# JuliaHealth/Thunderbolt.jl

Hardware: AMD Instinct MI355X
Metric: element-integrations/sec + DoF-updates/sec, 10M-hex Q1 monodomain (higher is better)
Workload: dtype f64

## Files before the change

### thunderbolt.jl_amd/csrc/tb_assembly.hip

```cpp
#include <hip/hip_runtime.h>

#include <cmath>
#include <cstring>
#include <type_traits>

#include "tb_elem.hpp"
#include "tb_forms.hpp"
#include "tb_hex8_sumfac.hpp"
#include "tb_internal.h"
#include "tb_math.hpp"

namespace tb {
using namespace tbk;

template <int NB> __host__ __device__ constexpr int sym_idx(int i, int j)
{
    return i <= j ? i * NB - (i * (i - 1)) / 2 + (j - i) : j * NB - (j * (j - 1)) / 2 + (i - j);
}

template <class E>
__device__ __forceinline__ void load_coords(const MeshView &m, int64_t cell, double (&x)[E::NV][3])
{
    int32_t nodes[E::NV];
    const int32_t *c = m.conn + cell * E::NV;
// ... 66 lines not shown
#pragma unroll
            for (int m = 0; m < 3; ++m)
#pragma unroll
                for (int l = 0; l < 3; ++l) H[m][l] = g.Jinv[m][0] * D[0][l] + g.Jinv[m][1] * D[1][l] + g.Jinv[m][2] * D[2][l];
#pragma unroll
            for (int m = 0; m < 3; ++m)
#pragma unroll
                for (int n = (SYM ? m : 0); n < 3; ++n)
                    G[m][n] = mw * (H[m][0] * g.Jinv[n][0] + H[m][1] * g.Jinv[n][1] + H[m][2] * g.Jinv[n][2]);
            if constexpr (SYM) { G[1][0] = G[0][1]; G[2][0] = G[0][2]; G[2][1] = G[1][2]; }
#pragma unroll
            for (int i = 0; i < NB; ++i) {
                double T[3];
#pragma unroll
                for (int m = 0; m < 3; ++m) T[m] = G[m][0] * tb.dN[q][i][0] + G[m][1] * tb.dN[q][i][1] + G[m][2] * tb.dN[q][i][2];
#pragma unroll
                for (int j = SYM ? i : 0; j < NB; ++j) {
                    double &k = Ke[SYM ? sym_idx<NB>(i, j) : i * NB + j];
                    k += tb.dN[q][j][0] * T[0];
                    k += tb.dN[q][j][1] * T[1];
                    k += tb.dN[q][j][2] * T[2];
                }
            }
        }
    }
    return ok;
}

template <class E>
__global__ void __launch_bounds__(256)
k_tabulate_spectral(const double *__restrict__ field, int64_t n_cells, double l0, double l1, double l2, double scale, double *__restrict__ dtab)
{
    const int64_t cell = (int64_t)blockIdx.x * blockDim.x + threadIdx.x;
    if (cell >= n_cells) return;
    constexpr int NB = E::NB;
    const Tables<E> &tb = g_tables<E>;
    double fc[NB * 9];
#pragma unroll
    for (int k = 0; k < NB * 9; ++k) fc[k] = field[cell * (NB * 9) + k];
#pragma unroll 1
    for (int q = 0; q < E::NQ; ++q) {
        double f[3] = {0, 0, 0}, s[3] = {0, 0, 0}, n[3] = {0, 0, 0};
#pragma unroll
        for (int a = 0; a < NB; ++a) {
            const double Na = tb.N[q][a];
#pragma unroll
            for (int d = 0; d < 3; ++d) {
                f[d] += Na * fc[9 * a + d];
                s[d] += Na * fc[9 * a + 3 + d];
                n[d] += Na * fc[9 * a + 6 + d];
            }
        }
        orthonormal_frame(f, s, n);
        double *o = dtab + (cell * E::NQ + q) * 6;
        int k = 0;
#pragma unroll
        for (int i = 0; i < 3; ++i)
#pragma unroll
            for (int j = i; j < 3; ++j) o[k++] = (l0 * f[i] * f[j] + l1 * s[i] * s[j] + l2 * n[i] * n[j]) * scale;
    }
}

template <class E>
__global__ void __launch_bounds__(256)
k_tabulate_isotropic(const double *__restrict__ field, int64_t n_cells, double scale, double *__restrict__ dtab)
{
    const int64_t cell = (int64_t)blockIdx.x * blockDim.x + threadIdx.x;
    if (cell >= n_cells) return;
    constexpr int NB = E::NB;
    const Tables<E> &tb = g_tables<E>;
    double fc[NB];
#pragma unroll
    for (int k = 0; k < NB; ++k) fc[k] = field[cell * NB + k];
    for (int q = 0; q < E::NQ; ++q) {
        double v = 0.0;
#pragma unroll
        for (int a = 0; a < NB; ++a) v += tb.N[q][a] * fc[a];
        v *= scale;
        double *o = dtab + (cell * E::NQ + q) * 6;
        o[0] = v; o[1] = 0.0; o[2] = 0.0; o[3] = v; o[4] = 0.0; o[5] = v;
    }
}

__device__ __forceinline__ double eval_source(const FormArgs &fa, const double (&xq)[3], int64_t cell, int q, int nq)
{
    switch (fa.src_kind) {
    case TB_SRC_CONST: return fa.p0;
    case TB_SRC_NORM_PLUS_T: return sqrt(xq[0] * xq[0] + xq[1] * xq[1] + xq[2] * xq[2]) + (fa.tslot ? fa.tslot[0] : fa.t);
    case TB_SRC_COS_EXP:
        return (fa.tslot ? fa.tslot[1] : fa.ct) * exp_b(-(xq[0] * xq[0] + xq[1] * xq[1] + xq[2] * xq[2]));
    case TB_SRC_TABULATED: return fa.table[cell * nq + q];
    }
    return 0.0;
}

template <class E>
__device__ __forceinline__ bool element_source(const double (&x)[E::NV][3], const FormArgs &fa, int64_t cell, double (&be)[E::NB])
{
    const Tables<E> &tb = g_tables<E>;
    GeoCoeffs<E> gc;
    geo_prepare(x, gc);
    bool ok = true;
#pragma unroll 1
    for (int q = 0; q < E::NQ; ++q) {
        Geom g;
        geometry_rt<E>(tb, q, gc, g);
        ok = ok && (g.dOmega > 0.0);
        double xq[3];
        geo_position(gc, tb, q, xq);
        const double fw = eval_source(fa, xq, cell, q, E::NQ) * g.dOmega;
#pragma unroll
        for (int j = 0; j < E::NB; ++j) be[j] += fw * tb.N[q][j];
    }
    return ok;
}

__device__ __forceinline__ void flag_neg_detj(Status *st, int64_t cell)
{
    st->neg_detj = 1;
    st->cell = cell;
}

template <class MapT>
__global__ void k_build_emap(const int32_t *__restrict__ cell_dofs, int64_t n_cells, int ndpc,
                             const int64_t *__restrict__ rowptr, const int32_t *__restrict__ colidx, MapT *__restrict__ emap,
                             Status *st)
{
    const int64_t tid = (int64_t)blockIdx.x * blockDim.x + threadIdx.x;
    if (tid >= n_cells * ndpc) return;
    const int64_t cell = tid % n_cells;
    const int i = (int)(tid / n_cells);
    const int32_t *d = cell_dofs + cell * ndpc;
    const int32_t row = d[i];
    const int64_t lo0 = rowptr[row], hi0 = rowptr[row + 1];
    for (int j = 0; j < ndpc; ++j) {
        const int32_t c = d[j];
        int64_t lo = lo0, hi = hi0;
        while (lo < hi) {
            const int64_t mid = (lo + hi) >> 1;
            if (colidx[mid] < c) lo = mid + 1; else hi = mid;
        }
        if (lo >= hi0 || colidx[lo] != c) { st->pattern_missing = 1; st->cell = cell; lo = lo0; }
        emap[(int64_t)(i * ndpc + j) * n_cells + cell] = (MapT)lo;
    }
}

template <class E, int FORM, bool FIELD, bool SYM, class MapT>
__global__ void __launch_bounds__(128)
k_matrix_direct(MeshView m, FormArgs fa, const MapT *__restrict__ emap, const int32_t *__restrict__ list, int64_t n,
                double *__restrict__ nz, int atomic, Status *st)
{
    constexpr int NB = E::NB;
    const int64_t tid = (int64_t)blockIdx.x * blockDim.x + threadIdx.x;
    if (tid >= n) return;
    const int64_t cell = list ? list[tid] : tid;
    double x[E::NV][3];
    load_coords<E>(m, cell, x);
    double Ke[SYM ? NB * (NB + 1) / 2 : NB * NB];
#pragma unroll
    for (int k = 0; k < (SYM ? NB * (NB + 1) / 2 : NB * NB); ++k) Ke[k] = 0.0;
    if (!element_matrix<E, FORM, FIELD, SYM>(x, fa, cell, Ke)) flag_neg_detj(st, cell);
    const MapT *mp = emap + cell;
#pragma unroll
    for (int i = 0; i < NB; ++i)
#pragma unroll
        for (int j = 0; j < NB; ++j) {
            const double v = Ke[SYM ? sym_idx<NB>(i, j) : i * NB + j];
            const int64_t k = (int64_t)mp[(int64_t)(i * NB + j) * m.n_cells];
            if (atomic) unsafeAtomicAdd(nz + k, v); else nz[k] += v;
        }
}

template <class E>
__global__ void __launch_bounds__(256)
// ... 94 lines not shown
        if (!element_matrix<E, FORM, FIELD, SYM>(x, fa, cell, Ke)) flag_neg_detj(st, cell);
#ifdef TB_ABLATION
        if (!(fa.debug & 1))
#endif
#pragma unroll
        for (int i = 0; i < NB; ++i) {
            if (ro[i] == 0xFFFF) continue;
            double *row = acc + ro[i];
#pragma unroll
            for (int j = 0; j < NB; ++j) unsafeAtomicAdd(row + cp[i * NB + j], Ke[SYM ? sym_idx<NB>(i, j) : i * NB + j]);
        }
        if (!more) break;
        e = en; cell = celln;
#pragma unroll
        for (int a_ = 0; a_ < E::NV; ++a_) { x[a_][0] = xn[a_][0]; x[a_][1] = xn[a_][1]; x[a_][2] = xn[a_][2]; }
    }
    __syncthreads();

#ifdef TB_ABLATION
    if (fa.debug & 1) { if (threadIdx.x == 0) nz[p] = acc[0] + Ke_sink(); }
    if (fa.debug & 2) return;
#endif
    const int half = threadIdx.x >> 5, hl = threadIdx.x & 31, nhalves = T >> 5;
#pragma unroll 4
    for (int s = half; s < nrows; s += nhalves) {
        const int64_t g0 = dnz[s];
        const uint2 ol = dol[s];
        double *dst = nz + g0;
        for (uint32_t k = hl; k < ol.y; k += 32) dst[k] = acc[ol.x + k];
    }
}

template <class E>
__global__ void __launch_bounds__(PATCH_MAX_THREADS)
k_vector_patch(MeshView m, FormArgs fa, PatchView pv, double *__restrict__ b, Status *st)
{
    extern __shared__ double acc[];
    const int T = blockDim.x;
    const int64_t p = blockIdx.x;
    const int64_t e0 = pv.elem_ptr[p], e1 = pv.elem_ptr[p + 1];
    const int64_t r0 = pv.row_ptr[p], r1 = pv.row_ptr[p + 1];
    const int nrows = (int)(r1 - r0);
    int64_t e = e0 + threadIdx.x;
    int64_t cell = 0;
    double x[E::NV][3];
    if (e < e1) { cell = pv.elem_cell[e]; load_coords<E>(m, cell, x); }
    for (int k = threadIdx.x; k < nrows; k += T) acc[k] = 0.0;
    __syncthreads();
    while (e < e1) {
        const int64_t en = e + T;
        const bool more = en < e1;
        int64_t celln = 0;
        double xn[E::NV][3];
        if (more) { celln = pv.elem_cell[en]; load_coords<E>(m, celln, xn); }
        uint16_t lr[E::NB];
        const uint16_t *lp = pv.elem_lrow + e * E::NB;
#pragma unroll
        for (int j = 0; j < E::NB; ++j) lr[j] = lp[j];
        double be[E::NB];
#pragma unroll
        for (int j = 0; j < E::NB; ++j) be[j] = 0.0;
        if (!element_source<E>(x, fa, cell, be)) flag_neg_detj(st, cell);
#pragma unroll
        for (int j = 0; j < E::NB; ++j)
            if (lr[j] != 0xFFFF) unsafeAtomicAdd(&acc[lr[j]], be[j]);
        if (!more) break;
        e = en; cell = celln;
#pragma unroll
        for (int a_ = 0; a_ < E::NV; ++a_) { x[a_][0] = xn[a_][0]; x[a_][1] = xn[a_][1]; x[a_][2] = xn[a_][2]; }
    }
    __syncthreads();
    for (int s = threadIdx.x; s < nrows; s += T) b[pv.row_dof[r0 + s]] = acc[s];
}

struct VecPatchView {
    const uint4 *hdr;
    const uint16_t *elem_ln;
    const int32_t *elem_cell;
    const double *pcoord;
    const int32_t *pdof;
    int max_nodes;
};

template <bool HALO>
__global__ void __launch_bounds__(256, 3)
k_vector_hex8_patch(FormArgs fa, VecPatchView pv, double *__restrict__ b, Status *st)
{
    extern __shared__ double lds[];
    constexpr int T = 256, NI = 2, NX = 13, ND = 3;
    const int tid = threadIdx.x;
    const uint4 h = pv.hdr[blockIdx.x];
    const int64_t e0 = h.x, n0 = h.y;
    const int nrows = (int)(h.z & 0xffff), nnodes = (int)(h.z >> 16), ne = (int)h.w;
    double *acc = lds;
    double *xs = lds + pv.max_nodes;
    uint4 lnv[NI];
#pragma unroll
    for (int k = 0; k < NI; ++k) lnv[k] = tid + k * T < ne ? ((const uint4 *)pv.elem_ln)[e0 + tid + k * T] : make_uint4(0, 0, 0, 0);
    const double *pc = pv.pcoord + 3 * n0;
    double xc[NX];
#pragma unroll
    for (int j = 0; j < NX; ++j) xc[j] = tid + j * T < 3 * nnodes ? pc[tid + j * T] : 0.0;
    const int32_t *pd = pv.pdof + n0;
    int32_t dofs[ND];
#pragma unroll
    for (int j = 0; j < ND; ++j) dofs[j] = tid + j * T < nrows ? pd[tid + j * T] : 0;
    for (int k = tid; k < nnodes; k += T) acc[k] = 0.0;
#pragma unroll
    for (int j = 0; j < NX; ++j) if (tid + j * T < 3 * nnodes) xs[tid + j * T] = xc[j];
    for (int k = tid + NX * T; k < 3 * nnodes; k += T) xs[k] = pc[k];
    __syncthreads();
#pragma unroll 1
    for (int it = 0, ei = tid; ei < ne; ++it, ei += T) {
        const uint4 l4 = it < NI ? lnv[0] : ((const uint4 *)pv.elem_ln)[e0 + ei];
#pragma unroll
        for (int k = 0; k + 1 < NI; ++k) lnv[k] = lnv[k + 1];
        const uint32_t ln[8] = {l4.x & 0xffffu, l4.x >> 16, l4.y & 0xffffu, l4.y >> 16, l4.z & 0xffffu, l4.z >> 16, l4.w & 0xffffu, l4.w >> 16};
        double x[8][3];
#pragma unroll
        for (int a = 0; a < 8; ++a) {
            const double *px = xs + 3 * ln[a];
            x[a][0] = px[0]; x[a][1] = px[1]; x[a][2] = px[2];
        }
        int64_t cell = 0;
        if (fa.src_kind == TB_SRC_TABULATED) cell = pv.elem_cell[e0 + ei];
        double be[8];
        if (!hex8_sf_source(x, [&](int q, const double(&xq)[3]) { return eval_source(fa, xq, cell, q, 8); }, be)) flag_neg_detj(st, pv.elem_cell[e0 + ei]);
#pragma unroll
        for (int a = 0; a < 8; ++a)
            if (!HALO || ln[a] < (uint32_t)nrows) unsafeAtomicAdd(acc + ln[a], be[a]);
    }
    __syncthreads();
#pragma unroll
    for (int j = 0; j < ND; ++j)
        if (tid + j * T < nrows) {
            if (HALO) b[dofs[j]] = acc[tid + j * T];
            else unsafeAtomicAdd(b + dofs[j], acc[tid + j * T]);
        }
    for (int k = tid + ND * T; k < nrows; k += T) {
        if (HALO) b[pd[k]] = acc[k];
        else unsafeAtomicAdd(b + pd[k], acc[k]);
    }
}


static inline unsigned nblocks(int64_t n, int bs) { return (unsigned)((n + bs - 1) / bs); }

int ensure_emap(tb_pattern *p)
{
    if (p->d_emap) return TB_OK;
    tb_mesh *m = p->mesh;
    tb_device *dev = m->dev;
    const int64_t n = m->n_cells * m->ndpc;
    p->map64 = p->nnz >= (int64_t)0x7fffffff;
    const size_t bytes = (size_t)m->n_cells * m->ndpc * m->ndpc * (p->map64 ? 8 : 4);
    TB_HIP(hipMalloc(&p->d_emap, bytes));
    int rc = reset_status(dev);
    if (rc) return rc;
    if (p->map64)
        hipLaunchKernelGGL(k_build_emap<int64_t>, dim3(nblocks(n, 256)), dim3(256), 0, dev->stream, m->d_cell_dofs, m->n_cells,
                           m->ndpc, p->d_rowptr, p->d_colidx, (int64_t *)p->d_emap, dev->d_status);
    else
        hipLaunchKernelGGL(k_build_emap<int32_t>, dim3(nblocks(n, 256)), dim3(256), 0, dev->stream, m->d_cell_dofs, m->n_cells,
                           m->ndpc, p->d_rowptr, p->d_colidx, (int32_t *)p->d_emap, dev->d_status);
    TB_HIP(hipGetLastError());
    return check_status(dev);
}

static PatchView make_patch_view(const tb_mesh *m, const tb_pattern *p)
{
    const PatchPlan *pp = m->patches.get();
    PatchView v{};
    v.elem_ptr = pp->d_elem_ptr; v.row_ptr = pp->d_row_ptr; v.elem_cell = pp->d_elem_cell;
    v.elem_lrow = pp->d_elem_lrow; v.row_dof = pp->d_row_dof;
    if (p) {
        const PatchMatPlan *pm = p->patch_mat.get();
        v.row_desc = pm->d_row_desc;
        v.elem_rowoff = pm->d_elem_rowoff;
        v.colpos = pm->d_colpos8 ? (const void *)pm->d_colpos8 : (const void *)pm->d_colpos16;
        v.lds_entries = pm->max_lds_entries;
        v.max_rows = pp->max_rows;
    }
    return v;
}

template <class E, int FORM, bool FIELD, bool SYM>
static int run_matrix(tb_form *f, tb_pattern *p, int strategy, double t, double *d_nz)
{
    tb_mesh *m = f->mesh;
    tb_device *dev = m->dev;
    const MeshView mv = make_view(m);
    const FormArgs fa = make_args(f, t);
    if (strategy == TB_STRATEGY_PATCH) {
        { int rc = ensure_patch_plans(m, p); if (rc) return rc; }
        const PatchView pv = make_patch_view(m, p);
        const size_t lds = (size_t)p->patch_mat->max_lds_entries * sizeof(double) + (size_t)m->patches->max_rows * 16;
        const int T = m->patches->threads;
        auto launch = [&](auto k) -> int {
            TB_HIP(hipFuncSetAttribute((const void *)k, hipFuncAttributeMaxDynamicSharedMemorySize, (int)lds));
            hipLaunchKernelGGL(k, dim3((unsigned)m->patches->n_patches), dim3(T), lds, dev->stream, mv, fa, pv, d_nz, dev->d_status);
            return TB_OK;
        };
        int rc;
        if (p->patch_mat->d_colpos8) rc = launch(k_matrix_patch<E, FORM, FIELD, SYM, uint8_t, 2>);
        else rc = launch(k_matrix_patch<E, FORM, FIELD, SYM, uint16_t, 2>);
        if (rc) return rc;
        TB_HIP(hipGetLastError());
        return TB_OK;
    }
    { int rc = ensure_emap(p); if (rc) return rc; }
    TB_HIP(hipMemsetAsync(d_nz, 0, (size_t)p->nnz * sizeof(double), dev->stream));
    auto go = [&](const int32_t *list, int64_t n, int atomic) -> int {
        if (n == 0) return TB_OK;
        if (p->map64)
            hipLaunchKernelGGL((k_matrix_direct<E, FORM, FIELD, SYM, int64_t>), dim3(nblocks(n, 128)), dim3(128), 0, dev->stream, mv, fa,
                               (const int64_t *)p->d_emap, list, n, d_nz, atomic, dev->d_status);
        else
            hipLaunchKernelGGL((k_matrix_direct<E, FORM, FIELD, SYM, int32_t>), dim3(nblocks(n, 128)), dim3(128), 0, dev->stream, mv, fa,
                               (const int32_t *)p->d_emap, list, n, d_nz, atomic, dev->d_status);
        TB_HIP(hipGetLastError());
        return TB_OK;
    };
// ... 792 lines not shown
    }
    __syncthreads();
    const int quarter = tid >> 4, ql = tid & 15;
    for (int s = quarter; s < nrows; s += T / 16) {
        const uint4 d = desc[s];
        const int64_t g0 = (int64_t)(((uint64_t)d.y << 32) | d.x);
        for (uint32_t k = ql; k < d.w; k += 16) {
            if constexpr (WK) nzK[g0 + k] = accK[d.z + k];
            if constexpr (WM) nzM[g0 + k] = accM[d.z + k];
        }
    }
}

bool tet4_patch_applicable(const tb_form *f, const tb_pattern *)
{
    static const bool legacy = getenv("TB_PATCH_KERNEL") && !strcmp(getenv("TB_PATCH_KERNEL"), "legacy");
    if (legacy) return false;
    const tb_mesh *m = f->mesh;
    if (m->field_kind != TB_TET4 || m->geom_kind != TB_TET4 || m->ncomp != 1 || f->qorder != 2 || f->has_cellset) return false;
    if (f->kind == TB_FORM_DIFFUSION) return !f->field;
    return f->kind == TB_FORM_MASS;
}

int launch_assemble_tet4_patch(tb_form *fK, tb_form *fM, tb_pattern *p, double t, double *d_nzK, double *d_nzM)
{
    tb_form *any = fK ? fK : fM;
    tb_mesh *m = any->mesh;
    tb_device *dev = m->dev;
    int rc = reset_status(dev);
    if (rc) return rc;
    const int nreg = fK && fM ? 2 : 1;
    rc = ensure_patch_fused(m, p, nreg);
    if (rc) return rc;
    const PatchPlan *pp = m->patches.get();
    const PatchFusedPlan *pf = p->patch_fused.get();
    if (!pf->d_hdr) { set_error("tetrahedron patch kernel: a patch exceeds the packed header (1023 rows / 2047 nodes / 2047 instances)"); return TB_ERR_UNSUPPORTED; }
    TetPatchView pv{pf->d_elem_ln, pf->d_elem_sig, pf->d_sigtab, pf->d_row_desc, pp->d_elem_cell, pf->max_lds_entries, pp->max_rows, pf->max_nodes};
    const size_t lds = (size_t)nreg * pv.kcap * sizeof(double) + (size_t)pv.max_rows * sizeof(RowDesc) + (size_t)pv.max_nodes * 3 * sizeof(double);
    const FormArgs aK = fK ? make_args(fK, t) : FormArgs{}, aM = fM ? make_args(fM, t) : FormArgs{};
    const bool fm = fM && fM->field;
    auto launch = [&](auto k) -> int {
        TB_HIP(hipFuncSetAttribute((const void *)k, hipFuncAttributeMaxDynamicSharedMemorySize, (int)lds));
        hipLaunchKernelGGL(k, dim3((unsigned)pp->n_patches), dim3(256), lds, dev->stream, aK, aM, pv, (const uint4 *)pf->d_hdr, pf->d_pcoord, d_nzK, d_nzM, dev->d_status);
        return TB_OK;
    };
    if (fK && fM) rc = fm ? launch(k_patch_tet4<true, true, true>) : launch(k_patch_tet4<true, true, false>);
    else if (fK) rc = launch(k_patch_tet4<true, false, false>);
    else rc = fm ? launch(k_patch_tet4<false, true, true>) : launch(k_patch_tet4<false, true, false>);
    if (rc) return rc;
    TB_HIP(hipGetLastError());
    return check_status(dev);
}

int launch_assemble_matrix(tb_form *f, tb_pattern *p, int strategy, double t, double *d_nz)
{
    tb_mesh *m = f->mesh;
    int rc = reset_status(m->dev);
    if (rc) return rc;
    if (strategy == TB_STRATEGY_ELEMENT && m->field_kind != TB_HEX27) strategy = TB_STRATEGY_PER_COLOR;
    if (strategy == TB_STRATEGY_PATCH && hex8_patch_applicable(f, p)) {
        rc = f->kind == TB_FORM_DIFFUSION ? launch_assemble_hex8_patch(f, nullptr, p, t, d_nz, nullptr) : launch_assemble_hex8_patch(nullptr, f, p, t, nullptr, d_nz);
        if (rc != TB_ERR_UNSUPPORTED) return rc;
        rc = reset_status(m->dev);
        if (rc) return rc;
    }
    if (strategy == TB_STRATEGY_PATCH && tet4_patch_applicable(f, p)) {
        rc = f->kind == TB_FORM_DIFFUSION ? launch_assemble_tet4_patch(f, nullptr, p, t, d_nz, nullptr) : launch_assemble_tet4_patch(nullptr, f, p, t, nullptr, d_nz);
        if (rc != TB_ERR_UNSUPPORTED) return rc;
        rc = reset_status(m->dev);
        if (rc) return rc;
    }
    if (m->field_kind == TB_HEX8 && f->qorder == 2) rc = run_matrix_form<Hex8<2>>(f, p, strategy, t, d_nz);
    else if (m->field_kind == TB_TET4 && f->qorder == 2) rc = run_matrix_form<Tet4<2>>(f, p, strategy, t, d_nz);
    else if (m->field_kind == TB_QUAD4 && f->qorder == 2) rc = run_matrix_form<Quad4<2>>(f, p, strategy, t, d_nz);
    else if (m->field_kind == TB_HEX27 && f->qorder == 3) rc = run_q2(f, p, strategy, t, d_nz, nullptr);
    else {
        set_error("matrix assembly: field kind %d with quadrature order %d not implemented", m->field_kind, f->qorder);
        return TB_ERR_UNSUPPORTED;
    }
    if (rc) return rc;
    return check_status(m->dev);
}

template <class E>
static int run_vector(tb_form *f, int strategy, double t, double *d_b)
{
    tb_mesh *m = f->mesh;
    tb_device *dev = m->dev;
    const MeshView mv = make_view(m);
    const FormArgs fa = make_args(f, t);
    static const bool legacy_vec = tune_env("TB_VECTOR_KERNEL") && !strcmp(tune_env("TB_VECTOR_KERNEL"), "legacy");
    if constexpr (std::is_same<E, Hex8<2>>::value) {
        if (!legacy_vec && !f->has_cellset && (strategy == TB_STRATEGY_PATCH || strategy == TB_STRATEGY_ATOMIC)) {
            const bool halo = strategy == TB_STRATEGY_PATCH;
            int rc = ensure_vec_patch_plan(m, halo);
            if (rc == TB_OK) {
                const VecPatchPlan *vp = m->vpatches[halo].get();
                const VecPatchView pv{(const uint4 *)vp->d_hdr, vp->d_elem_ln, vp->d_elem_cell, vp->d_pcoord, vp->d_pdof, vp->max_nodes};
                const size_t lds = (size_t)vp->max_nodes * 4 * sizeof(double);
                if (!halo) TB_HIP(hipMemsetAsync(d_b, 0, (size_t)m->ndofs * sizeof(double), dev->stream));
                if (halo) {
                    TB_HIP(hipFuncSetAttribute((const void *)k_vector_hex8_patch<true>, hipFuncAttributeMaxDynamicSharedMemorySize, (int)lds));
                    hipLaunchKernelGGL(k_vector_hex8_patch<true>, dim3((unsigned)vp->n_patches), dim3(256), lds, dev->stream, fa, pv, d_b, dev->d_status);
                } else {
                    TB_HIP(hipFuncSetAttribute((const void *)k_vector_hex8_patch<false>, hipFuncAttributeMaxDynamicSharedMemorySize, (int)lds));
                    hipLaunchKernelGGL(k_vector_hex8_patch<false>, dim3((unsigned)vp->n_patches), dim3(256), lds, dev->stream, fa, pv, d_b, dev->d_status);
                }
                TB_HIP(hipGetLastError());
                return TB_OK;
            }
            if (rc != TB_ERR_UNSUPPORTED) return rc;
        }
    }
    if (strategy == TB_STRATEGY_PATCH) {
        { int rc = ensure_patch_plans(m, nullptr); if (rc) return rc; }
        const PatchView pv = make_patch_view(m, nullptr);
        const int T = m->patches->threads;
        hipLaunchKernelGGL((k_vector_patch<E>), dim3((unsigned)m->patches->n_patches), dim3(T),
                           (size_t)m->patches->max_rows * sizeof(double), dev->stream, mv, fa, pv, d_b, dev->d_status);
        TB_HIP(hipGetLastError());
        return TB_OK;
    }
    if (strategy == TB_STRATEGY_ELEMENT) {
        if (!m->ea) { int rc = build_ea_plan(m); if (rc) return rc; }
        hipLaunchKernelGGL((k_vector_direct<E>), dim3(nblocks(m->n_cells, 256)), dim3(256), 0, dev->stream, mv, fa,
                           (const int32_t *)nullptr, m->n_cells, d_b, m->ea->d_ea, 2, dev->d_status);
        TB_HIP(hipGetLastError());
        hipLaunchKernelGGL(k_ea_gather, dim3(nblocks(m->ndofs, 256)), dim3(256), 0, dev->stream, m->ea->d_ptr, m->ea->d_src,
                           m->ea->d_ea, m->ndofs, d_b);
        TB_HIP(hipGetLastError());
        return TB_OK;
    }
    TB_HIP(hipMemsetAsync(d_b, 0, (size_t)m->ndofs * sizeof(double), dev->stream));
    if (strategy == TB_STRATEGY_ATOMIC) {
        hipLaunchKernelGGL((k_vector_direct<E>), dim3(nblocks(m->n_cells, 256)), dim3(256), 0, dev->stream, mv, fa,
                           (const int32_t *)nullptr, m->n_cells, d_b, (double *)nullptr, 0, dev->d_status);
        TB_HIP(hipGetLastError());
        return TB_OK;
    }
    if (strategy == TB_STRATEGY_PER_COLOR) {
        if (!m->colors) { int rc = build_color_plan(m); if (rc) return rc; }
        for (int c = 0; c < m->colors->ncolors; ++c) {
            const int64_t n = m->colors->offsets[c + 1] - m->colors->offsets[c];
            if (!n) continue;
            hipLaunchKernelGGL((k_vector_direct<E>), dim3(nblocks(n, 256)), dim3(256), 0, dev->stream, mv, fa,
                               (const int32_t *)(m->colors->d_cells + m->colors->offsets[c]), n, d_b, (double *)nullptr, 1, dev->d_status);
            TB_HIP(hipGetLastError());
        }
        return TB_OK;
    }
    set_error("vector assembly: unknown strategy %d", strategy);
    return TB_ERR_UNSUPPORTED;
}

int launch_assemble_vector(tb_form *f, int strategy, double t, double *d_b)
{
    tb_mesh *m = f->mesh;
    int rc = reset_status(m->dev);
    if (rc) return rc;
    if (m->ncomp != 1) { set_error("source assembly needs a scalar field"); return TB_ERR_UNSUPPORTED; }
    if (m->field_kind == TB_HEX8 && f->qorder == 2) rc = run_vector<Hex8<2>>(f, strategy, t, d_b);
    else if (m->field_kind == TB_HEX8 && f->qorder == 3) rc = run_vector<Hex8<3>>(f, strategy, t, d_b);
    else if (m->field_kind == TB_TET4 && f->qorder == 2) rc = run_vector<Tet4<2>>(f, strategy, t, d_b);
    else if (m->field_kind == TB_QUAD4 && f->qorder == 2) rc = run_vector<Quad4<2>>(f, strategy, t, d_b);
    else if (m->field_kind == TB_HEX27 && f->qorder == 3) rc = run_q2(f, nullptr, strategy, t, nullptr, d_b);
    else {
        set_error("vector assembly: field kind %d with quadrature order %d not implemented", m->field_kind, f->qorder);
        return TB_ERR_UNSUPPORTED;
    }
    if (rc) return rc;
    return check_status(m->dev);
}

}
```

### thunderbolt.jl_amd/csrc/tb_hex8_sumfac.hpp

```cpp
#pragma once
#include "tb_elem.hpp"

namespace tbk {

struct SF {
    static constexpr double g = 0.5773502691896258;
    static constexpr double p = 0.5 * (1.0 + g), m = 0.5 * (1.0 - g);
    TB_HD static constexpr int bit(int a, int d) { return Hex8<2>::sgn(a, d) > 0 ? 1 : 0; }
    TB_HD static constexpr double f(int b, int qb) { return b == qb ? p : m; }
    TB_HD static constexpr double w(int t, int qb) { return t == 1 ? p * m : (t == 0 ? f(0, qb) * f(0, qb) : f(1, qb) * f(1, qb)); }
    TB_HD static constexpr int ty(int i, int j, int d) { return bit(i, d) + bit(j, d); }
    TB_HD static constexpr int sg(int i, int j, int d, int e) { return Hex8<2>::sgn(i, d) * Hex8<2>::sgn(j, e); }
};

__device__ __forceinline__ double sf_rcp(double y)
{
    double r = __builtin_amdgcn_rcp(y);
    r = fma(fma(-y, r, 1.0), r, r);
    r = fma(fma(-y, r, 1.0), r, r);
    return r;
}

template <bool WANT_K, bool FENCE, bool DIAG = false, bool ISO = false, class DFn>
__device__ __forceinline__ bool hex8_sf_geometry(const double (&x)[8][3], DFn &&Dq, double (&G)[8][6], double (&dq)[8], double sfac = -0.25)
// ... 42 lines not shown
            const double s = sfac * sf_rcp(det);
            double H[3][3];
#pragma unroll
            for (int a = 0; a < 3; ++a) {
                if constexpr (DIAG) {
                    H[a][0] = A[a][0] * D[0]; H[a][1] = A[a][1] * D[3]; H[a][2] = A[a][2] * D[5];
                } else {
                    H[a][0] = A[a][0] * D[0] + A[a][1] * D[1] + A[a][2] * D[2];
                    H[a][1] = A[a][0] * D[1] + A[a][1] * D[3] + A[a][2] * D[4];
                    H[a][2] = A[a][0] * D[2] + A[a][1] * D[4] + A[a][2] * D[5];
                }
            }
            int k = 0;
#pragma unroll
            for (int a = 0; a < 3; ++a)
#pragma unroll
                for (int b = a; b < 3; ++b) G[q][k++] = s * (H[a][0] * A[b][0] + H[a][1] * A[b][1] + H[a][2] * A[b][2]);
        }
        if constexpr (FENCE) __builtin_amdgcn_sched_barrier(0);
    }
    return ok;
}

template <int COMP, int DIR>
__device__ __forceinline__ void hex8_sf_diag(const double (&G)[8][6], double (&Y)[3][3])
{
    constexpr int E = DIR == 0 ? 1 : 0, F = DIR == 2 ? 1 : 2;
    double S[2][2];
#pragma unroll
    for (int qf = 0; qf < 2; ++qf)
#pragma unroll
        for (int qe = 0; qe < 2; ++qe) S[qf][qe] = G[(qe << E) | (qf << F)][COMP] + G[(qe << E) | (qf << F) | (1 << DIR)][COMP];
    double T[3][2];
#pragma unroll
    for (int qf = 0; qf < 2; ++qf) {
        T[0][qf] = fma(SF::w(0, 1), S[qf][1], SF::w(0, 0) * S[qf][0]);
        T[1][qf] = SF::w(1, 0) * (S[qf][0] + S[qf][1]);
        T[2][qf] = fma(SF::w(2, 1), S[qf][1], SF::w(2, 0) * S[qf][0]);
    }
#pragma unroll
    for (int te = 0; te < 3; ++te) {
        Y[te][0] = fma(SF::w(0, 1), T[te][1], SF::w(0, 0) * T[te][0]);
        Y[te][1] = SF::w(1, 0) * (T[te][0] + T[te][1]);
        Y[te][2] = fma(SF::w(2, 1), T[te][1], SF::w(2, 0) * T[te][0]);
    }
}
template <int COMP, int D, int E>
__device__ __forceinline__ void hex8_sf_cross(const double (&G)[8][6], double (&X)[2][2][3])
{
    constexpr int F = 3 - D - E;
    double A1[2][2][2];
#pragma unroll
    for (int qe = 0; qe < 2; ++qe)
#pragma unroll
        for (int qf = 0; qf < 2; ++qf) {
            const double g0 = G[(qe << E) | (qf << F)][COMP], g1 = G[(qe << E) | (qf << F) | (1 << D)][COMP];
            A1[0][qe][qf] = fma(SF::f(0, 1), g1, SF::f(0, 0) * g0);
            A1[1][qe][qf] = fma(SF::f(1, 1), g1, SF::f(1, 0) * g0);
        }
    double B1[2][2][2];
#pragma unroll
    for (int a = 0; a < 2; ++a)
#pragma unroll
        for (int qf = 0; qf < 2; ++qf) {
            B1[a][0][qf] = fma(SF::f(0, 1), A1[a][1][qf], SF::f(0, 0) * A1[a][0][qf]);
            B1[a][1][qf] = fma(SF::f(1, 1), A1[a][1][qf], SF::f(1, 0) * A1[a][0][qf]);
        }
#pragma unroll
    for (int a = 0; a < 2; ++a)
#pragma unroll
        for (int b = 0; b < 2; ++b) {
            X[a][b][0] = fma(SF::w(0, 1), B1[a][b][1], SF::w(0, 0) * B1[a][b][0]);
            X[a][b][1] = SF::w(1, 0) * (B1[a][b][0] + B1[a][b][1]);
            X[a][b][2] = fma(SF::w(2, 1), B1[a][b][1], SF::w(2, 0) * B1[a][b][0]);
        }
}

template <class FFn>
__device__ __forceinline__ bool hex8_sf_source(const double (&x)[8][3], FFn &&F, double (&be)[8])
{
    GeoCoeffs<Hex8<2>> gc;
    geo_prepare(x, gc);
    constexpr double gg = SF::g;
    double c0[4][3], c1[4][3], c2[4][3], xq[8][3];
#pragma unroll
    for (int i = 0; i < 3; ++i) {
#pragma unroll
        for (int b = 0; b < 2; ++b) {
            const double sb = b ? gg : -gg;
            const double a0 = fma(gc.c[6][i], sb, gc.c[1][i]), a1 = fma(gc.c[7][i], sb, gc.c[4][i]);
            c0[0 + 2 * b][i] = fma(a1, -gg, a0); c0[1 + 2 * b][i] = fma(a1, gg, a0);
            const double b0 = fma(gc.c[5][i], sb, gc.c[2][i]);
            c1[0 + 2 * b][i] = fma(a1, -gg, b0); c1[1 + 2 * b][i] = fma(a1, gg, b0);
            const double d0 = fma(gc.c[5][i], sb, gc.c[3][i]), d1 = fma(gc.c[7][i], sb, gc.c[6][i]);
            c2[0 + 2 * b][i] = fma(d1, -gg, d0); c2[1 + 2 * b][i] = fma(d1, gg, d0);
            const double p0 = fma(gc.c[3][i], sb, gc.c[0][i]);
#pragma unroll
            for (int e = 0; e < 2; ++e) {
                const double se = e ? gg : -gg;
                const double r0 = fma(b0, se, p0), r1 = fma(a1, se, a0);
                xq[0 + 2 * e + 4 * b][i] = fma(r1, -gg, r0);
                xq[1 + 2 * e + 4 * b][i] = fma(r1, gg, r0);
            }
        }
    }
    bool ok = true;
    double fw[8];
#pragma unroll
    for (int q = 0; q < 8; ++q) {
        const int q1 = q & 1, q2 = (q >> 1) & 1, q3 = q >> 2;
        const double(&u)[3] = c0[q2 + 2 * q3];
        const double(&v)[3] = c1[q1 + 2 * q3];
        const double(&z)[3] = c2[q1 + 2 * q2];
        const double det = u[0] * (v[1] * z[2] - z[1] * v[2]) + u[1] * (z[0] * v[2] - v[0] * z[2]) + u[2] * (v[0] * z[1] - z[0] * v[1]);
        ok = ok && (det > 0.0);
        fw[q] = F(q, xq[q]) * det;
    }
    double A1[2][2][2];
#pragma unroll
    for (int q2 = 0; q2 < 2; ++q2)
#pragma unroll
        for (int q3 = 0; q3 < 2; ++q3) {
            const double f0 = fw[2 * q2 + 4 * q3], f1 = fw[1 + 2 * q2 + 4 * q3];
            A1[0][q2][q3] = fma(SF::f(0, 1), f1, SF::f(0, 0) * f0);
            A1[1][q2][q3] = fma(SF::f(1, 1), f1, SF::f(1, 0) * f0);
        }
    double B1[2][2][2];
#pragma unroll
    for (int b1 = 0; b1 < 2; ++b1)
#pragma unroll
        for (int q3 = 0; q3 < 2; ++q3) {
            B1[b1][0][q3] = fma(SF::f(0, 1), A1[b1][1][q3], SF::f(0, 0) * A1[b1][0][q3]);
            B1[b1][1][q3] = fma(SF::f(1, 1), A1[b1][1][q3], SF::f(1, 0) * A1[b1][0][q3]);
        }
#pragma unroll
    for (int j = 0; j < 8; ++j) {
        const int b1 = SF::bit(j, 0), b2 = SF::bit(j, 1), b3 = SF::bit(j, 2);
        be[j] = fma(SF::f(b3, 1), B1[b1][b2][1], SF::f(b3, 0) * B1[b1][b2][0]);
    }
    return ok;
}

struct Hex8SFK {
    double Y11[3][3], Y22[3][3], Y33[3][3];
    double X12[2][2][3], X13[2][2][3], X23[2][2][3];
};

__device__ __forceinline__ void hex8_sf_contract(const double (&G)[8][6], Hex8SFK &c)
{
    hex8_sf_diag<0, 0>(G, c.Y11);
    hex8_sf_diag<3, 1>(G, c.Y22);
    hex8_sf_diag<5, 2>(G, c.Y33);
    hex8_sf_cross<1, 0, 1>(G, c.X12);
    hex8_sf_cross<2, 0, 2>(G, c.X13);
    hex8_sf_cross<4, 1, 2>(G, c.X23);
}

__device__ __forceinline__ double hex8_sf_pair(bool pa, double a, bool pb, double b)
{
    return pa ? (pb ? a + b : a - b) : (pb ? b - a : -(a + b));
}
__device__ __forceinline__ double hex8_sf_entry(const Hex8SFK &c, int i, int j)
{
    const int t0 = SF::ty(i, j, 0), t1 = SF::ty(i, j, 1), t2 = SF::ty(i, j, 2);
    const int bi0 = SF::bit(i, 0), bi1 = SF::bit(i, 1), bi2 = SF::bit(i, 2);
    const int bj0 = SF::bit(j, 0), bj1 = SF::bit(j, 1), bj2 = SF::bit(j, 2);
#ifndef TB_SF_ENTRY_TREE
    double v = SF::sg(i, j, 0, 0) > 0 ? c.Y11[t1][t2] : -c.Y11[t1][t2];
    v += SF::sg(i, j, 1, 1) > 0 ? c.Y22[t0][t2] : -c.Y22[t0][t2];
    v += SF::sg(i, j, 2, 2) > 0 ? c.Y33[t0][t1] : -c.Y33[t0][t1];
    v += SF::sg(i, j, 0, 1) > 0 ? c.X12[bj0][bi1][t2] : -c.X12[bj0][bi1][t2];
    v += SF::sg(j, i, 0, 1) > 0 ? c.X12[bi0][bj1][t2] : -c.X12[bi0][bj1][t2];
    v += SF::sg(i, j, 0, 2) > 0 ? c.X13[bj0][bi2][t1] : -c.X13[bj0][bi2][t1];
    v += SF::sg(j, i, 0, 2) > 0 ? c.X13[bi0][bj2][t1] : -c.X13[bi0][bj2][t1];
    v += SF::sg(i, j, 1, 2) > 0 ? c.X23[bj1][bi2][t0] : -c.X23[bj1][bi2][t0];
    v += SF::sg(j, i, 1, 2) > 0 ? c.X23[bi1][bj2][t0] : -c.X23[bi1][bj2][t0];
    return v;
#else
    const double a0 = hex8_sf_pair(SF::sg(i, j, 0, 0) > 0, c.Y11[t1][t2], SF::sg(i, j, 1, 1) > 0, c.Y22[t0][t2]);
    const double a1 = hex8_sf_pair(SF::sg(i, j, 2, 2) > 0, c.Y33[t0][t1], SF::sg(i, j, 0, 1) > 0, c.X12[bj0][bi1][t2]);
    const double a2 = hex8_sf_pair(SF::sg(j, i, 0, 1) > 0, c.X12[bi0][bj1][t2], SF::sg(i, j, 0, 2) > 0, c.X13[bj0][bi2][t1]);
    const double a3 = hex8_sf_pair(SF::sg(j, i, 0, 2) > 0, c.X13[bi0][bj2][t1], SF::sg(i, j, 1, 2) > 0, c.X23[bj1][bi2][t0]);
    const double x9 = c.X23[bi1][bj2][t0];
    const double s = (a0 + a1) + (a2 + a3);
    return SF::sg(j, i, 1, 2) > 0 ? s + x9 : s - x9;
#endif
}

__device__ __forceinline__ void hex8_sf_mass(const double (&d)[8], double (&Z)[3][3][3])
{
    double U[3][2][2];
#pragma unroll
    for (int q2 = 0; q2 < 2; ++q2)
#pragma unroll
        for (int q3 = 0; q3 < 2; ++q3) {
            const double d0 = d[2 * q2 + 4 * q3], d1 = d[1 + 2 * q2 + 4 * q3];
            U[0][q2][q3] = fma(SF::w(0, 1), d1, SF::w(0, 0) * d0);
            U[1][q2][q3] = SF::w(1, 0) * (d0 + d1);
            U[2][q2][q3] = fma(SF::w(2, 1), d1, SF::w(2, 0) * d0);
        }
    double V[3][3][2];
#pragma unroll
    for (int t1 = 0; t1 < 3; ++t1)
#pragma unroll
        for (int q3 = 0; q3 < 2; ++q3) {
            V[t1][0][q3] = fma(SF::w(0, 1), U[t1][1][q3], SF::w(0, 0) * U[t1][0][q3]);
            V[t1][1][q3] = SF::w(1, 0) * (U[t1][0][q3] + U[t1][1][q3]);
            V[t1][2][q3] = fma(SF::w(2, 1), U[t1][1][q3], SF::w(2, 0) * U[t1][0][q3]);
        }
#pragma unroll
    for (int t1 = 0; t1 < 3; ++t1)
#pragma unroll
        for (int t2 = 0; t2 < 3; ++t2) {
            Z[t1][t2][0] = fma(SF::w(0, 1), V[t1][t2][1], SF::w(0, 0) * V[t1][t2][0]);
            Z[t1][t2][1] = SF::w(1, 0) * (V[t1][t2][0] + V[t1][t2][1]);
            Z[t1][t2][2] = fma(SF::w(2, 1), V[t1][t2][1], SF::w(2, 0) * V[t1][t2][0]);
        }
// ... 4 lines not shown
```

Measured before the change: 11.38 billion.

## Specialize hex8 vector patch kernel on source kind and cut register pressure

Templates the hex8 vector-assembly patch kernel on source kind so the per-quadrature switch is resolved at compile time, and hoists the time lookup out of the loop. It drops register prefetch buffers for element-local indices and dof lists, reloads indices at scatter time, and restructures the sum-factorized source evaluation to process one z-slab at a time so fewer values are live. Launch bounds go from 3 to 4 blocks per CU. In the halo variant, LDS atomics are serialized wave by wave with block barriers, which adds synchronization in exchange for ordered accumulation.

```diff
diff --git a/thunderbolt.jl_amd/csrc/tb_assembly.hip b/thunderbolt.jl_amd/csrc/tb_assembly.hip
--- a/thunderbolt.jl_amd/csrc/tb_assembly.hip
+++ b/thunderbolt.jl_amd/csrc/tb_assembly.hip
@@ -172,14 +172,32 @@
     }
 }
 
+template <int KIND>
+__device__ __forceinline__ double eval_source_k(const FormArgs &fa, double tv, const double (&xq)[3], int64_t cell, int q, int nq)
+{
+    static_assert(KIND == TB_SRC_CONST || KIND == TB_SRC_NORM_PLUS_T || KIND == TB_SRC_COS_EXP || KIND == TB_SRC_TABULATED, "unknown source kind");
+    if constexpr (KIND == TB_SRC_CONST) return fa.p0;
+    else if constexpr (KIND == TB_SRC_NORM_PLUS_T) return sqrt(xq[0] * xq[0] + xq[1] * xq[1] + xq[2] * xq[2]) + tv;
+    else if constexpr (KIND == TB_SRC_COS_EXP)
+        return tv * exp_b(-(xq[0] * xq[0] + xq[1] * xq[1] + xq[2] * xq[2]));
+    else return fa.table[cell * nq + q];
+}
+
+template <int KIND>
+__device__ __forceinline__ double source_time(const FormArgs &fa)
+{
+    if constexpr (KIND == TB_SRC_NORM_PLUS_T) return fa.tslot ? fa.tslot[0] : fa.t;
+    else if constexpr (KIND == TB_SRC_COS_EXP) return fa.tslot ? fa.tslot[1] : fa.ct;
+    else return 0.0;
+}
+
 __device__ __forceinline__ double eval_source(const FormArgs &fa, const double (&xq)[3], int64_t cell, int q, int nq)
 {
     switch (fa.src_kind) {
-    case TB_SRC_CONST: return fa.p0;
-    case TB_SRC_NORM_PLUS_T: return sqrt(xq[0] * xq[0] + xq[1] * xq[1] + xq[2] * xq[2]) + (fa.tslot ? fa.tslot[0] : fa.t);
-    case TB_SRC_COS_EXP:
-        return (fa.tslot ? fa.tslot[1] : fa.ct) * exp_b(-(xq[0] * xq[0] + xq[1] * xq[1] + xq[2] * xq[2]));
-    case TB_SRC_TABULATED: return fa.table[cell * nq + q];
+    case TB_SRC_CONST: return eval_source_k<TB_SRC_CONST>(fa, 0.0, xq, cell, q, nq);
+    case TB_SRC_NORM_PLUS_T: return eval_source_k<TB_SRC_NORM_PLUS_T>(fa, source_time<TB_SRC_NORM_PLUS_T>(fa), xq, cell, q, nq);
+    case TB_SRC_COS_EXP: return eval_source_k<TB_SRC_COS_EXP>(fa, source_time<TB_SRC_COS_EXP>(fa), xq, cell, q, nq);
+    case TB_SRC_TABULATED: return eval_source_k<TB_SRC_TABULATED>(fa, 0.0, xq, cell, q, nq);
     }
     return 0.0;
 }
@@ -440,62 +458,68 @@
     int max_nodes;
 };
 
-template <bool HALO>
-__global__ void __launch_bounds__(256, 3)
+template <bool HALO, int KIND>
+__global__ void __launch_bounds__(256, 4)
 k_vector_hex8_patch(FormArgs fa, VecPatchView pv, double *__restrict__ b, Status *st)
 {
     extern __shared__ double lds[];
-    constexpr int T = 256, NI = 2, NX = 13, ND = 3;
+    constexpr int T = 256, NX = 13;
     const int tid = threadIdx.x;
     const uint4 h = pv.hdr[blockIdx.x];
     const int64_t e0 = h.x, n0 = h.y;
     const int nrows = (int)(h.z & 0xffff), nnodes = (int)(h.z >> 16), ne = (int)h.w;
     double *acc = lds;
     double *xs = lds + pv.max_nodes;
-    uint4 lnv[NI];
-#pragma unroll
-    for (int k = 0; k < NI; ++k) lnv[k] = tid + k * T < ne ? ((const uint4 *)pv.elem_ln)[e0 + tid + k * T] : make_uint4(0, 0, 0, 0);
+    const uint4 *eln = (const uint4 *)pv.elem_ln + e0;
     const double *pc = pv.pcoord + 3 * n0;
     double xc[NX];
 #pragma unroll
     for (int j = 0; j < NX; ++j) xc[j] = tid + j * T < 3 * nnodes ? pc[tid + j * T] : 0.0;
     const int32_t *pd = pv.pdof + n0;
-    int32_t dofs[ND];
-#pragma unroll
-    for (int j = 0; j < ND; ++j) dofs[j] = tid + j * T < nrows ? pd[tid + j * T] : 0;
     for (int k = tid; k < nnodes; k += T) acc[k] = 0.0;
 #pragma unroll
     for (int j = 0; j < NX; ++j) if (tid + j * T < 3 * nnodes) xs[tid + j * T] = xc[j];
     for (int k = tid + NX * T; k < 3 * nnodes; k += T) xs[k] = pc[k];
+    const double tv = source_time<KIND>(fa);
     __syncthreads();
 #pragma unroll 1
-    for (int it = 0, ei = tid; ei < ne; ++it, ei += T) {
-        const uint4 l4 = it < NI ? lnv[0] : ((const uint4 *)pv.elem_ln)[e0 + ei];
-#pragma unroll
-        for (int k = 0; k + 1 < NI; ++k) lnv[k] = lnv[k + 1];
-        const uint32_t ln[8] = {l4.x & 0xffffu, l4.x >> 16, l4.y & 0xffffu, l4.y >> 16, l4.z & 0xffffu, l4.z >> 16, l4.w & 0xffffu, l4.w >> 16};
-        double x[8][3];
-#pragma unroll
-        for (int a = 0; a < 8; ++a) {
-            const double *px = xs + 3 * ln[a];
-            x[a][0] = px[0]; x[a][1] = px[1]; x[a][2] = px[2];
-        }
-        int64_t cell = 0;
-        if (fa.src_kind == TB_SRC_TABULATED) cell = pv.elem_cell[e0 + ei];
+    for (int ei = tid; HALO ? ei - tid < ne : ei < ne; ei += T) {
+        const bool on = !HALO || ei < ne;
         double be[8];
-        if (!hex8_sf_source(x, [&](int q, const double(&xq)[3]) { return eval_source(fa, xq, cell, q, 8); }, be)) flag_neg_detj(st, pv.elem_cell[e0 + ei]);
-#pragma unroll
-        for (int a = 0; a < 8; ++a)
-            if (!HALO || ln[a] < (uint32_t)nrows) unsafeAtomicAdd(acc + ln[a], be[a]);
-    }
-    __syncthreads();
-#pragma unroll
-    for (int j = 0; j < ND; ++j)
-        if (tid + j * T < nrows) {
-            if (HALO) b[dofs[j]] = acc[tid + j * T];
-            else unsafeAtomicAdd(b + dofs[j], acc[tid + j * T]);
-        }
-    for (int k = tid + ND * T; k < nrows; k += T) {
+        if (on) {
+            const uint4 l4 = eln[ei];
+            const uint32_t ln[8] = {l4.x & 0xffffu, l4.x >> 16, l4.y & 0xffffu, l4.y >> 16, l4.z & 0xffffu, l4.z >> 16, l4.w & 0xffffu, l4.w >> 16};
+            double x[8][3];
+#pragma unroll
+            for (int a = 0; a < 8; ++a) {
+                const double *px = xs + 3 * ln[a];
+                x[a][0] = px[0]; x[a][1] = px[1]; x[a][2] = px[2];
+            }
+            int64_t cell = 0;
+            if constexpr (KIND == TB_SRC_TABULATED) cell = pv.elem_cell[e0 + ei];
+            if (!hex8_sf_source(x, [&](int q, const double(&xq)[3]) { return eval_source_k<KIND>(fa, tv, xq, cell, q, 8); }, be)) flag_neg_detj(st, pv.elem_cell[e0 + ei]);
+        }
+        auto scatter = [&]() {
+            int es = ei;
+            asm volatile("" : "+v"(es));
+            const uint4 s4 = eln[es];
+            const uint32_t sn[8] = {s4.x & 0xffffu, s4.x >> 16, s4.y & 0xffffu, s4.y >> 16, s4.z & 0xffffu, s4.z >> 16, s4.w & 0xffffu, s4.w >> 16};
+#pragma unroll
+            for (int a = 0; a < 8; ++a)
+                if (!HALO || sn[a] < (uint32_t)nrows) unsafeAtomicAdd(acc + sn[a], be[a]);
+        };
+        if constexpr (HALO) {
+#pragma unroll 1
+            for (int w = 0; w < T / 64; ++w) {
+                if (on && (tid >> 6) == w) scatter();
+                __syncthreads();
+            }
+        } else {
+            scatter();
+        }
+    }
+    if constexpr (!HALO) __syncthreads();
+    for (int k = tid; k < nrows; k += T) {
         if (HALO) b[pd[k]] = acc[k];
         else unsafeAtomicAdd(b + pd[k], acc[k]);
     }
@@ -1454,6 +1478,19 @@
     return check_status(m->dev);
 }
 
+template <bool HALO, int KIND>
+static int launch_vector_hex8_patch_inst(int64_t n_patches, size_t lds, tb_device *dev, const FormArgs &fa, const VecPatchView &pv, double *d_b)
+{
+    hipLaunchKernelGGL((k_vector_hex8_patch<HALO, KIND>), dim3((unsigned)n_patches), dim3(256), lds, dev->stream, fa, pv, d_b, dev->d_status);
+    TB_HIP(hipGetLastError());
+    return TB_OK;
+}
+template <int KIND>
+static int launch_vector_hex8_patch(bool halo, int64_t n_patches, size_t lds, tb_device *dev, const FormArgs &fa, const VecPatchView &pv, double *d_b)
+{
+    return halo ? launch_vector_hex8_patch_inst<true, KIND>(n_patches, lds, dev, fa, pv, d_b) : launch_vector_hex8_patch_inst<false, KIND>(n_patches, lds, dev, fa, pv, d_b);
+}
+
 template <class E>
 static int run_vector(tb_form *f, int strategy, double t, double *d_b)
 {
@@ -1471,15 +1508,13 @@
                 const VecPatchView pv{(const uint4 *)vp->d_hdr, vp->d_elem_ln, vp->d_elem_cell, vp->d_pcoord, vp->d_pdof, vp->max_nodes};
                 const size_t lds = (size_t)vp->max_nodes * 4 * sizeof(double);
                 if (!halo) TB_HIP(hipMemsetAsync(d_b, 0, (size_t)m->ndofs * sizeof(double), dev->stream));
-                if (halo) {
-                    TB_HIP(hipFuncSetAttribute((const void *)k_vector_hex8_patch<true>, hipFuncAttributeMaxDynamicSharedMemorySize, (int)lds));
-                    hipLaunchKernelGGL(k_vector_hex8_patch<true>, dim3((unsigned)vp->n_patches), dim3(256), lds, dev->stream, fa, pv, d_b, dev->d_status);
-                } else {
-                    TB_HIP(hipFuncSetAttribute((const void *)k_vector_hex8_patch<false>, hipFuncAttributeMaxDynamicSharedMemorySize, (int)lds));
-                    hipLaunchKernelGGL(k_vector_hex8_patch<false>, dim3((unsigned)vp->n_patches), dim3(256), lds, dev->stream, fa, pv, d_b, dev->d_status);
-                }
-                TB_HIP(hipGetLastError());
-                return TB_OK;
+                rc = fa.src_kind == TB_SRC_CONST         ? launch_vector_hex8_patch<TB_SRC_CONST>(halo, vp->n_patches, lds, dev, fa, pv, d_b)
+                     : fa.src_kind == TB_SRC_NORM_PLUS_T ? launch_vector_hex8_patch<TB_SRC_NORM_PLUS_T>(halo, vp->n_patches, lds, dev, fa, pv, d_b)
+                     : fa.src_kind == TB_SRC_COS_EXP     ? launch_vector_hex8_patch<TB_SRC_COS_EXP>(halo, vp->n_patches, lds, dev, fa, pv, d_b)
+                     : fa.src_kind == TB_SRC_TABULATED   ? launch_vector_hex8_patch<TB_SRC_TABULATED>(halo, vp->n_patches, lds, dev, fa, pv, d_b)
+                                                         : TB_ERR_BAD_ARG;
+                if (rc == TB_ERR_BAD_ARG) set_error("vector assembly: unknown source kind %d", fa.src_kind);
+                return rc;
             }
             if (rc != TB_ERR_UNSUPPORTED) return rc;
         }
diff --git a/thunderbolt.jl_amd/csrc/tb_hex8_sumfac.hpp b/thunderbolt.jl_amd/csrc/tb_hex8_sumfac.hpp
--- a/thunderbolt.jl_amd/csrc/tb_hex8_sumfac.hpp
+++ b/thunderbolt.jl_amd/csrc/tb_hex8_sumfac.hpp
@@ -148,57 +148,60 @@
     GeoCoeffs<Hex8<2>> gc;
     geo_prepare(x, gc);
     constexpr double gg = SF::g;
-    double c0[4][3], c1[4][3], c2[4][3], xq[8][3];
-#pragma unroll
-    for (int i = 0; i < 3; ++i) {
-#pragma unroll
-        for (int b = 0; b < 2; ++b) {
-            const double sb = b ? gg : -gg;
+    double c2[4][3];
+#pragma unroll
+    for (int i = 0; i < 3; ++i)
+#pragma unroll
+        for (int e = 0; e < 2; ++e) {
+            const double se = e ? gg : -gg;
+            const double d0 = fma(gc.c[5][i], se, gc.c[3][i]), d1 = fma(gc.c[7][i], se, gc.c[6][i]);
+            c2[0 + 2 * e][i] = fma(d1, -gg, d0); c2[1 + 2 * e][i] = fma(d1, gg, d0);
+        }
+    bool ok = true;
+    double B1[2][2][2];
+#pragma unroll
+    for (int b = 0; b < 2; ++b) {
+        const double sb = b ? gg : -gg;
+        double c0[2][3], c1[2][3], xq[4][3];
+#pragma unroll
+        for (int i = 0; i < 3; ++i) {
             const double a0 = fma(gc.c[6][i], sb, gc.c[1][i]), a1 = fma(gc.c[7][i], sb, gc.c[4][i]);
-            c0[0 + 2 * b][i] = fma(a1, -gg, a0); c0[1 + 2 * b][i] = fma(a1, gg, a0);
+            c0[0][i] = fma(a1, -gg, a0); c0[1][i] = fma(a1, gg, a0);
             const double b0 = fma(gc.c[5][i], sb, gc.c[2][i]);
-            c1[0 + 2 * b][i] = fma(a1, -gg, b0); c1[1 + 2 * b][i] = fma(a1, gg, b0);
-            const double d0 = fma(gc.c[5][i], sb, gc.c[3][i]), d1 = fma(gc.c[7][i], sb, gc.c[6][i]);
-            c2[0 + 2 * b][i] = fma(d1, -gg, d0); c2[1 + 2 * b][i] = fma(d1, gg, d0);
+            c1[0][i] = fma(a1, -gg, b0); c1[1][i] = fma(a1, gg, b0);
             const double p0 = fma(gc.c[3][i], sb, gc.c[0][i]);
 #pragma unroll
             for (int e = 0; e < 2; ++e) {
                 const double se = e ? gg : -gg;
                 const double r0 = fma(b0, se, p0), r1 = fma(a1, se, a0);
-                xq[0 + 2 * e + 4 * b][i] = fma(r1, -gg, r0);
-                xq[1 + 2 * e + 4 * b][i] = fma(r1, gg, r0);
+                xq[0 + 2 * e][i] = fma(r1, -gg, r0);
+                xq[1 + 2 * e][i] = fma(r1, gg, r0);
             }
         }
-    }
-    bool ok = true;
-    double fw[8];
-#pragma unroll
-    for (int q = 0; q < 8; ++q) {
-        const int q1 = q & 1, q2 = (q >> 1) & 1, q3 = q >> 2;
-        const double(&u)[3] = c0[q2 + 2 * q3];
-        const double(&v)[3] = c1[q1 + 2 * q3];
-        const double(&z)[3] = c2[q1 + 2 * q2];
-        const double det = u[0] * (v[1] * z[2] - z[1] * v[2]) + u[1] * (z[0] * v[2] - v[0] * z[2]) + u[2] * (v[0] * z[1] - z[0] * v[1]);
-        ok = ok && (det > 0.0);
-        fw[q] = F(q, xq[q]) * det;
-    }
-    double A1[2][2][2];
-#pragma unroll
-    for (int q2 = 0; q2 < 2; ++q2)
-#pragma unroll
-        for (int q3 = 0; q3 < 2; ++q3) {
-            const double f0 = fw[2 * q2 + 4 * q3], f1 = fw[1 + 2 * q2 + 4 * q3];
-            A1[0][q2][q3] = fma(SF::f(0, 1), f1, SF::f(0, 0) * f0);
-            A1[1][q2][q3] = fma(SF::f(1, 1), f1, SF::f(1, 0) * f0);
-        }
-    double B1[2][2][2];
-#pragma unroll
-    for (int b1 = 0; b1 < 2; ++b1)
-#pragma unroll
-        for (int q3 = 0; q3 < 2; ++q3) {
-            B1[b1][0][q3] = fma(SF::f(0, 1), A1[b1][1][q3], SF::f(0, 0) * A1[b1][0][q3]);
-            B1[b1][1][q3] = fma(SF::f(1, 1), A1[b1][1][q3], SF::f(1, 0) * A1[b1][0][q3]);
-        }
+        double fw[4];
+#pragma unroll
+        for (int k = 0; k < 4; ++k) {
+            const int q1 = k & 1, q2 = k >> 1;
+            const double(&u)[3] = c0[q2];
+            const double(&v)[3] = c1[q1];
+            const double(&z)[3] = c2[q1 + 2 * q2];
+            const double det = u[0] * (v[1] * z[2] - z[1] * v[2]) + u[1] * (z[0] * v[2] - v[0] * z[2]) + u[2] * (v[0] * z[1] - z[0] * v[1]);
+            ok = ok && (det > 0.0);
+            fw[k] = F(k + 4 * b, xq[k]) * det;
+        }
+        double A1[2][2];
+#pragma unroll
+        for (int q2 = 0; q2 < 2; ++q2) {
+            const double f0 = fw[2 * q2], f1 = fw[1 + 2 * q2];
+            A1[0][q2] = fma(SF::f(0, 1), f1, SF::f(0, 0) * f0);
+            A1[1][q2] = fma(SF::f(1, 1), f1, SF::f(1, 0) * f0);
+        }
+#pragma unroll
+        for (int b1 = 0; b1 < 2; ++b1) {
+            B1[b1][0][b] = fma(SF::f(0, 1), A1[b1][1], SF::f(0, 0) * A1[b1][0]);
+            B1[b1][1][b] = fma(SF::f(1, 1), A1[b1][1], SF::f(1, 0) * A1[b1][0]);
+        }
+    }
 #pragma unroll
     for (int j = 0; j < 8; ++j) {
         const int b1 = SF::bit(j, 0), b2 = SF::bit(j, 1), b3 = SF::bit(j, 2);
```

Result: faster. 11.56 billion (median of 6 runs) (+1.5%).
